# cboin1996/avddpg

Hardware: AMD Instinct MI355X
Metric: env-steps/sec + DDPG updates/sec, 4096x5-vehicle platoons (higher is better)
Workload: dtype f32-class (fp16 hi+lo operand pairs on the 16-bit matrix cores, f32 accumulate)

## Files before the change

### avddpg_amd/csrc/fsplit.hip

```cpp
#include <type_traits>

#include "fset_common.h"
#include "anchor.h"
#include "smooth.h"

namespace avd {
namespace fsplit {
using namespace fset;

struct ActorS {
    static constexpr int K = 256, KP = 256, NFT = 8, NKS = 16, LD = 264, NGT = 9, KG = 288;
    static constexpr bool critic = false;
};
struct CriticS {
    static constexpr int K = 304, KP = 320, NFT = 10, NKS = 19, LD = 312, NGT = 10, KG = 320;
    static constexpr bool critic = true;
};
constexpr int NGT_MAX = 10;

template <int I, int N, class F>
__device__ __forceinline__ void static_for(F&& f) {
    if constexpr (I < N) {
        f(std::integral_constant<int, I>{});
        static_for<I + 1, N>(f);
// ... 350 lines not shown
    b -= a.n_zero;
    const int which = b >= a.n_pack;
    pack_x_role<S>(a.pk, which, b - which * a.n_pack, a.pa.fflag + 4 * ((long)a.n_prep1 + b));
}

enum HeadMode { OUT_TANH = 0, OUT_TD = 1, HEAD_BOTH = 5, OUT_TANH_SAVE = 6 };
struct HeadArgs {
    unsigned long long* stamp;
    NetP net;
    int n_agents, n_sets;
    const f16x8* xf;
    const float* act;
    const float* act2;
    const float* r;
    const float* yin;
    const float* aw;
    float* out;
    unsigned* sm;
    float* g3;
    float* dmu;
    float* part_s;
    float* part_s2;
    float* part_m;
    float* tz;
    float gamma, high, inv_n;
    int* bad;
    int abl;
};
#ifndef HEAD_FAST
#define HEAD_FAST 5
#define HEAD_SLOW 3
#endif

template <int S, class NET, int MODE, bool HP = false, class... H>
__global__ __launch_bounds__(NT) void head_kernel(const HeadArgs p, H... hp) {
    constexpr int K = NET::K, NKS = NET::NKS, NFT = NET::NFT, LD = NET::LD;
    constexpr int NTH = NT;
    constexpr bool BOTH = (MODE == HEAD_BOTH);
    static_assert(!BOTH || NET::critic, "HEAD_BOTH is a critic mode");
    __shared__ __attribute__((aligned(16))) f16 wimg[2][H2 * LD];
    __shared__ __attribute__((aligned(16))) float b2s[H2];
    __shared__ __attribute__((aligned(16))) float c3s[H2];
    __shared__ __attribute__((aligned(16))) unsigned waps[BOTH ? 48 : 4];
    const int tid = threadIdx.x, w = tid >> 6, lane = tid & 63, r = lane & 31, h = lane >> 5, q = w >> 1, rh = w & 1;
    const int set = blockIdx.x % p.n_sets, j0 = blockIdx.x / p.n_sets, J = gridDim.x / p.n_sets, P = p.n_agents / p.n_sets;
#ifdef AVD_STAMP
    unsigned long long hacc[4] = {0, 0, 0, 0}, hlast = __builtin_amdgcn_s_memtime();
    const unsigned long long hstart = hlast;
#define HSTAMP(i) { const unsigned long long t_ = __builtin_amdgcn_s_memtime(); hacc[i] += t_ - hlast; hlast = t_; }
#else
#define HSTAMP(i)
#endif
    const float* vec = p.net.vec + (long)set * VEC;
    const f16x8* wf1 = p.net.wf1h + (long)set * NGT_MAX * 64 + lane;
    const f32x16 zero16 = {};
    const int ntile = j0 < P ? (P - j0 + J - 1) / J : 0;
    const int row = 32 * rh + r;
    f16x8 nx = {};
    float na = 0.f, nb = 0.f, ny = 0.f, nw = 1.f;
    auto fetch_in = [&](int k) {
        const int agent = (j0 + k * J) * p.n_sets + set;
        const long ri = (long)agent * TILE + row;
        nx = p.xf[2 * ri + h];
        if (NET::critic) na = p.act[ri];
        if (BOTH) nb = p.act2[ri];
        if (MODE == OUT_TD) ny = p.r[ri];
        if (BOTH) ny = p.yin[ri];
        if (BOTH && p.aw) nw = p.aw[agent];
    };
    constexpr int FAST = HEAD_FAST, SLOW = HEAD_SLOW, PERIOD = 2 * (FAST + SLOW);
    const int qs = __builtin_amdgcn_readfirstlane(q);
    const int cnt = qs < 2 ? FAST : SLOW, start = qs < 2 ? qs * FAST : 2 * FAST + (qs - 2) * SLOW;
    int k = start, pos = 0;
    auto next_tile = [&](int kk, int pp) { return pp + 1 == cnt ? kk + PERIOD - cnt + 1 : kk + 1; };
    const float SW = vec[2 * H2 + 1], d3 = vec[2 * H2];
    const float vb = vec[tid & (H2 - 1)], vc = vec[H2 + (tid & (H2 - 1))];
    unsigned wv = 0;
// ... 272 lines not shown
            if constexpr (HP) {
                if (h == 0) p.out[ri] = ty + hp_of(set, hp...).gamma * z;
            } else {
                if (h == 0) p.out[ri] = ty + p.gamma * z;
            }
        }
        HSTAMP(2);
#ifdef AVD_STAMP
        if (blockIdx.x == 16 && lane == 0 && p.stamp && (w == 0 || w == 4) && ui < 28)
            p.stamp[64 + (w >> 2) * 28 + ui] = hlast - hstart;
#endif
    }
#ifdef AVD_STAMP
    if (blockIdx.x == 16 && lane == 0 && p.stamp)
        for (int i = 0; i < 4; ++i) p.stamp[w * 8 + i] = hacc[i];
#endif
    if (watch >= 0x7f800000u) atomicOr(p.bad, 1);
    if (BOTH) {
#pragma unroll
        for (int o = 1; o < 32; o <<= 1) {
            Dacc += __shfl_xor(Dacc, o), Lacc += __shfl_xor(Lacc, o);
            Dacc2 += __shfl_xor(Dacc2, o), Lacc2 += __shfl_xor(Lacc2, o);
        }
#pragma unroll
        for (int o = 1; o < 64; o <<= 1) gmax = fmaxf(gmax, __shfl_xor(gmax, o));
        if (lane == 0) {
            const long slot = (long)blockIdx.x * 8 + w;
            p.part_m[slot] = gmax;
            p.part_s[slot * 2] = Dacc, p.part_s[slot * 2 + 1] = Lacc;
            p.part_s2[slot * 2] = Dacc2, p.part_s2[slot * 2 + 1] = Lacc2;
        }
    }
}

struct SeedArgs {
    int n_agents, n_sets;
    const float *dmu, *tz;
    float high;
    float *g3, *part_m, *part_s;
};
__global__ __launch_bounds__(NT) void actor_seed_kernel(const SeedArgs p) {
    const int tid = threadIdx.x, w = tid >> 6, lane = tid & 63;
    const int set = blockIdx.x % p.n_sets, j0 = blockIdx.x / p.n_sets, J = gridDim.x / p.n_sets, P = p.n_agents / p.n_sets;
    float gmax = 0.f, D = 0.f;
    for (int pi = j0 + w * J; pi < P; pi += 8 * J) {
        const long ri = (long)(pi * p.n_sets + set) * TILE + lane;
        const float t = p.tz[ri], g = p.dmu[ri] * p.high * (1.f - t * t);
        p.g3[ri] = g;
        gmax = fmaxf(gmax, fabsf(g));
        D += g;
    }
#pragma unroll
    for (int o = 1; o < 64; o <<= 1) gmax = fmaxf(gmax, __shfl_xor(gmax, o)), D += __shfl_xor(D, o);
    if (lane == 0) {
        p.part_m[(long)blockIdx.x * 8 + w] = gmax;
        p.part_s[((long)blockIdx.x * 8 + w) * 2] = D, p.part_s[((long)blockIdx.x * 8 + w) * 2 + 1] = 0.f;
    }
}

__device__ __forceinline__ float set_gscale(const float* part_m, int set, int n_sets, int J, float* red) {
    const int tid = threadIdx.x;
    float m = 0.f;
    for (int i = tid; i < J * 8; i += NT) m = fmaxf(m, part_m[((long)(i >> 3) * n_sets + set) * 8 + (i & 7)]);
#pragma unroll
    for (int o = 1; o < 64; o <<= 1) m = fmaxf(m, __shfl_xor(m, o));
    if ((tid & 63) == 0) red[tid >> 6] = m;
    __syncthreads();
    m = fmaxf(fmaxf(fmaxf(red[0], red[1]), fmaxf(red[2], red[3])), fmaxf(fmaxf(red[4], red[5]), fmaxf(red[6], red[7])));
    int e = 0;
    if (m > 0.f && !not_finite(m)) (void)frexpf(m, &e);
    const int k = e > 100 ? -100 : (e < -100 ? 100 : -e);
    return __uint_as_float(__builtin_amdgcn_readfirstlane(__float_as_uint(ldexpf(1.f, k))));
}

__device__ __forceinline__ unsigned mask_pair(unsigned d, int j, unsigned mj) { return __umul24(d & (0x10001u << j), mj); }
__device__ __forceinline__ void mask_chunk16(unsigned w, int c, unsigned m, uint4& lo, uint4& hi) {
    const unsigned d = w >> (8 * (c & 1));
    lo.x = mask_pair(d, 0, m), lo.y = mask_pair(d, 1, m >> 1), lo.z = mask_pair(d, 2, m >> 2), lo.w = mask_pair(d, 3, m >> 3);
    hi.x = mask_pair(d, 4, m >> 4), hi.y = mask_pair(d, 5, m >> 5), hi.z = mask_pair(d, 6, m >> 6), hi.w = mask_pair(d, 7, m >> 7);
}
__device__ __forceinline__ unsigned mask_one(float g3, bool signed_) { return signed_ && g3 < 0.f ? 0xbc00u : 0x3c00u; }

struct DwArgs {
    NetP net;
    int n_agents, n_sets;
    const float* x;
    const float* act;
    const float* g3;
    const float* part_m;
    const unsigned* sm;
    float* partG;
    int abl;
    unsigned long long* stamp;
};
template <int S, class NET>
__global__ __launch_bounds__(NT) void dw_kernel(const DwArgs p) {
    constexpr int KG = NET::KG, LDZ = 160;
    constexpr int XC = NET::critic ? 2 : 1;
    __shared__ __attribute__((aligned(16))) f16 smimg[2][TILE * LDZ];
    __shared__ __attribute__((aligned(16))) f16x8 fq[2][TILE * 2];
    __shared__ __attribute__((aligned(16))) f16x8 fa[2][TILE * 2];
    __shared__ float gred[8];
    const int tid = threadIdx.x, w = tid >> 6, lane = tid & 63, r = lane & 31, h = lane >> 5;
    const int set = blockIdx.x % p.n_sets, j0 = blockIdx.x / p.n_sets, J = gridDim.x / p.n_sets, P = p.n_agents / p.n_sets;
    float gsc;
    const f16x8* wf1 = p.net.wf1h + (long)set * NGT_MAX * 64 + lane;
    const int xt = NET::critic ? 8 + (w >> 2) : 8, xrh = NET::critic ? (w >> 1) & 1 : (w >> 2) & 1, xc0 = NET::critic ? 2 * (w & 1) : (w & 3);
    const f16x8 wf0 = wf1[64 * w], wfx = wf1[64 * xt];
    f32x16 G0[4], G1[XC];
    const f32x16 zero16 = {};
#pragma unroll
    for (int c = 0; c < 4; ++c) G0[c] = zero16;
#pragma unroll
    for (int c = 0; c < XC; ++c) G1[c] = zero16;

    const int srow = tid >> 3, sch = tid & 7, frow = tid >> 1, fh = tid & 1;
    unsigned ma = 0, mb = 0;
    float sx[4] = {0.f, 0.f, 0.f, 0.f}, sg = 0.f, sa = 0.f, ga = 0.f, gb = 0.f;
    auto fetch_m = [&](int pl, unsigned& m, float& g) {
        const long ri = (long)(((FSPLIT_ABL(p.abl) & 1) ? j0 : pl) * p.n_sets + set) * TILE + srow;
        m = p.sm[ri * 4 + (sch >> 1)];
        g = p.g3[ri];
    };
    auto fetch_x = [&](int pl) {
        if (pl >= P || tid >= 2 * TILE) return;
        const long ri = (long)(pl * p.n_sets + set) * TILE + frow;
        load_x<S>(p.x, ri, sx);
        sg = p.g3[ri];
        if (NET::critic) sa = p.act[ri];
    };
    auto stage_m = [&](int buf, unsigned m, float g) {
        uint4* dst = (uint4*)(smimg[buf] + srow * LDZ + 16 * sch);
        mask_chunk16(m, sch, mask_one(g, true), dst[0], dst[1]);
    };
    auto stage_x = [&](int pl, int buf) {
        if (pl >= P) return;
// ... 82 lines not shown
            __builtin_amdgcn_sched_barrier(0);
        }
        stage_m(buf ^ 1, m, g);
#pragma unroll
        for (int s = 0; s < 2; ++s) {
            const f16x8 hi = fragh(ah[4 * s], ah[4 * s + 1], ah[4 * s + 2], ah[4 * s + 3]);
            const f16x8 lo = fragh(al[4 * s], al[4 * s + 1], al[4 * s + 2], al[4 * s + 3]);
#pragma unroll
            for (int c = 0; c < XC; ++c) {
                f16x8 bx;
#pragma unroll
                for (int hf = 0; hf < 2; ++hf) {
                    const int R0 = 32 * xrh + 16 * s + 8 * hf + 4 * (g4 >> 1);
                    const f16x4 t = read_tr(smimg[buf] + (R0 + q) * LDZ + 32 * (xc0 + c) + 16 * (g4 & 1) + 4 * pp);
#pragma unroll
                    for (int j = 0; j < 4; ++j) bx[4 * hf + j] = t[j];
                }
                G1[c] = mfmah(hi, bx, G1[c]);
                G1[c] = mfmah(lo, bx, G1[c]);
            }
        }
        __builtin_amdgcn_sched_group_barrier(0x100, 4 * XC, 0);
#pragma unroll
        for (int i = 0; i < 4 * XC; ++i) {
            __builtin_amdgcn_sched_group_barrier(0x008, 1, 0);
            __builtin_amdgcn_sched_group_barrier(0x002, 6, 0);
        }
        __builtin_amdgcn_sched_group_barrier(0x200, 2, 0);
        __builtin_amdgcn_sched_barrier(0);
    };
    if (j0 < P) fetch_m(j0, ma, ga);
    fetch_x(j0);
    if (j0 + J < P) fetch_m(j0 + J, mb, gb);
    gsc = set_gscale(p.part_m, set, p.n_sets, J, gred);
    stage_m(0, ma, ga), stage_x(j0, 0);
    __syncthreads();
#ifdef AVD_STAMP
    unsigned long long tacc[4] = {0, 0, 0, 0}, tlast = __builtin_amdgcn_s_memtime();
#define STAMP(i) { const unsigned long long t_ = __builtin_amdgcn_s_memtime(); tacc[i] += t_ - tlast; tlast = t_; }
#else
#define STAMP(i)
#endif
    for (int pi = j0; pi < P; pi += 2 * J) {
        fetch_x(pi + J);
        if (pi + 2 * J < P) fetch_m(pi + 2 * J, ma, ga);
        STAMP(0);
        compute(0, mb, gb);
        STAMP(1);
        stage_x(pi + J, 1);
        STAMP(2);
        if (!(FSPLIT_ABL(p.abl) & 2)) __syncthreads();
        STAMP(3);
        if (pi + J < P) {
            fetch_x(pi + 2 * J);
            if (pi + 3 * J < P) fetch_m(pi + 3 * J, mb, gb);
            STAMP(0);
            compute(1, ma, ga);
            STAMP(1);
            stage_x(pi + 2 * J, 0);
            STAMP(2);
            if (!(FSPLIT_ABL(p.abl) & 2)) __syncthreads();
            STAMP(3);
        }
    }
#ifdef AVD_STAMP
    if (p.stamp && blockIdx.x == 16 && lane == 0)
        for (int i = 0; i < 4; ++i) p.stamp[w * 8 + i] = tacc[i];
#endif
    const float dsc = 1.f / (gsc * S1);
    float* comb = (float*)&smimg[0][0];
    const int cidx = NET::critic ? 2 * (w >> 2) + (w & 1) : (w & 3);
    if (xrh == 1) {
#pragma unroll
        for (int c = 0; c < XC; ++c)
#pragma unroll
            for (int k = 0; k < 16; ++k) comb[((cidx * XC + c) * 16 + k) * 64 + lane] = G1[c][k];
    }
    __syncthreads();
#pragma unroll
    for (int c = 0; c < 4; ++c) {
        float* dst = p.partG + ((long)blockIdx.x * KG + 32 * w) * H2 + 32 * c + r;
#pragma unroll
        for (int k = 0; k < 16; ++k) dst[(long)acc_row(k, h) * H2] = G0[c][k] * dsc;
    }
    if (xrh == 0) {
#pragma unroll
        for (int c = 0; c < XC; ++c) {
            float* dst = p.partG + ((long)blockIdx.x * KG + 32 * xt) * H2 + 32 * (xc0 + c) + r;
#pragma unroll
            for (int k = 0; k < 16; ++k) dst[(long)acc_row(k, h) * H2] = (G1[c][k] + comb[((cidx * XC + c) * 16 + k) * 64 + lane]) * dsc;
        }
    }
}

struct DxArgs {
    NetP net;
    int n_agents, n_sets;
    const f16x8* xfh;
    const float* act;
    int L_cWa, L_cba;
    const float* g3;
    const float* part_m;
    const unsigned* sm;
    float* partV;
    int abl;
    unsigned long long* stamp;
};
template <int S, class NET>
__global__ __launch_bounds__(NT) void dx_kernel(const DxArgs p) {
    constexpr int KP = NET::KP, LDZ = 136;
    constexpr float VSH = 1.f / 32.f;
    __shared__ __attribute__((aligned(16))) f16 smimg[2][TILE * LDZ];
    __shared__ __attribute__((aligned(16))) f16 xt[3][2][32 * 32];
    __shared__ __attribute__((aligned(16))) float g3s[3][TILE];
    __shared__ float gred[8];
    const int tid = threadIdx.x, w = __builtin_amdgcn_readfirstlane(tid >> 6), lane = tid & 63, r = lane & 31, h = lane >> 5, ft = w;
    const int set = blockIdx.x % p.n_sets, j0 = blockIdx.x / p.n_sets, J = gridDim.x / p.n_sets, P = p.n_agents / p.n_sets;
    const f32x16 zero16 = {};
    f16x8 wch[8], wcl[8];
    {
        const long at = ((long)set * KP + 32 * ft + r) * H2 + 8 * h;
#pragma unroll
        for (int s = 0; s < 8; ++s) wch[s] = *(const f16x8*)(p.net.Wchi + at + 16 * s), wcl[s] = *(const f16x8*)(p.net.Wclo + at + 16 * s);
    }
    const float swc = __uint_as_float(__builtin_amdgcn_readfirstlane(__float_as_uint(p.net.vec[(long)set * VEC + 2 * H2 + 2])));
    float gv, vs;
    const f16x8 wf = p.net.wf1h[((long)set * NGT_MAX + ft) * 64 + lane];
    f32x16 V = zero16;
    for (int i = tid; i < 3 * 2 * 32 * 32; i += NT) {
        const int k = (i >> 5) & 31;
        (&xt[0][0][0])[i] = (f16)(k == 8 ? 1.f : 0.f);
    }
    const int srow = tid >> 3, sch = tid & 7;
    unsigned dm = 0;
    float gn = 0.f, gs = 0.f;
    auto fetch = [&](int pl) {
        if (FSPLIT_ABL(p.abl) & 1) pl = j0;
        const long agent = (long)pl * p.n_sets + set;
        dm = p.sm[(agent * TILE + srow) * 4 + (sch >> 1)];
        if (NET::critic) gs = p.g3[agent * TILE + srow];
        if (tid < TILE) gn = p.g3[agent * TILE + tid];
    };
    auto stage = [&](int buf, int slot) {
        uint4* dst = (uint4*)(smimg[buf] + srow * LDZ + 16 * sch);
        mask_chunk16(dm, sch, mask_one(gs, NET::critic), dst[0], dst[1]);
        if (tid < TILE) g3s[slot][tid] = (NET::critic ? fabsf(gn) : gn) * gv;
    };
    f16x8 xfn0 = {}, xfn1 = {};
    auto fetch_x = [&](int pl) {
// ... 92 lines not shown
        if constexpr (has_prev) v_product(vh1, vl1, xb1);
        read_a(buf, 1, smf);
        read_img(xt[slot][0], xb0);
        dc1 = dc_product(smf);
        p11 = mfmah(xf1, wf, zero16);
        backward(slot, 0, dc0, p10, vh0, vl0);
        stage(buf ^ 1, nslot);
        stage_x(nslot);
        xf0 = xfn0, xf1 = xfn1;
        fetch(nn), fetch_x(nn);
        __builtin_amdgcn_sched_group_barrier(0x100, 16, 0);
#pragma unroll
        for (int i = 0; i < (has_prev ? 21 : 17); ++i) {
            __builtin_amdgcn_sched_group_barrier(0x008, 1, 0);
            __builtin_amdgcn_sched_group_barrier(0x002, 6, 0);
            __builtin_amdgcn_sched_group_barrier(0x200, 1, 0);
        }
        __builtin_amdgcn_sched_barrier(0);
        v_product(vh0, vl0, xb0);
        DXSTAMP(2);
        if (!(FSPLIT_ABL(p.abl) & 2)) __syncthreads();
        DXSTAMP(3);
    };
    unsigned dm0 = 0;
    float gn0 = 0.f, gs0 = 0.f;
    f16x8 xfa = {}, xfb = {};
    if (j0 < P) {
        fetch(j0), fetch_x(j0);
        dm0 = dm, gn0 = gn, gs0 = gs, xfa = xfn0, xfb = xfn1;
        const int n1 = j0 + J < P ? j0 + J : j0;
        fetch(n1), fetch_x(n1);
    }
    {
        const float gsc = set_gscale(p.part_m, set, p.n_sets, J, gred);
        gv = gsc * VSH, vs = gsc * swc * VSH;
    }
    if (j0 < P) {
        const unsigned dm1 = dm;
        const float gn1 = gn, gs1 = gs;
        const f16x8 xfc = xfn0, xfd = xfn1;
        dm = dm0, gn = gn0, gs = gs0, xfn0 = xfa, xfn1 = xfb;
        stage(0, 0), stage_x(0);
        xf0 = xfn0, xf1 = xfn1;
        dm = dm1, gn = gn1, gs = gs1, xfn0 = xfc, xfn1 = xfd;
    }
    __syncthreads();
    if (j0 < P) {
        iteration(std::false_type{}, j0, 0, 0);
        int buf = 1, slot = 1, pi = j0 + J;
        for (; pi < P; pi += J, buf ^= 1, slot = slot == 2 ? 0 : slot + 1) iteration(std::true_type{}, pi, buf, slot);
        const int pslot = slot == 0 ? 2 : slot - 1;
        f16x8 xb1[2];
        unsigned vh1[8], vl1[8];
        read_img(xt[pslot][1], xb1);
        backward(pslot, 1, dc1, p11, vh1, vl1);
        v_product(vh1, vl1, xb1);
    }
#ifdef AVD_STAMP
    if (p.stamp && blockIdx.x == 16 && lane == 0)
        for (int i = 0; i < 4; ++i) p.stamp[w * 8 + i] = dacc[i];
#endif
    const float ivs = 1.f / vs;
    if (r < 16) {
        float* pv = p.partV + ((long)blockIdx.x * KP + 32 * ft) * 16 + r;
#pragma unroll
        for (int k = 0; k < 16; ++k) pv[(long)acc_row(k, h) * 16] = V[k] * ivs;
    }
}

template <int S>
__global__ __launch_bounds__(NT) void dxa_kernel(const DxArgs p) {
    typedef CriticS NET;
    constexpr int KP = NET::KP;
    constexpr float VSH = 1.f / 32.f;
    __shared__ __attribute__((aligned(16))) float ga[8][2][2][32];
    __shared__ float comb[8][64][2];
    __shared__ float gred[8];
    const int tid = threadIdx.x, w = __builtin_amdgcn_readfirstlane(tid >> 6), lane = tid & 63, r = lane & 31, h = lane >> 5;
    const int rh = w & 1, ftl = (w >> 1) & 1, par = w >> 2;
    const int set = blockIdx.x % p.n_sets, j0 = blockIdx.x / p.n_sets, J = gridDim.x / p.n_sets, P = p.n_agents / p.n_sets;
    const f32x16 zero16 = {};
    const int ft = 8 + ftl, f = 32 * ftl + r;
    f16x8 wch[8], wcl[8];
    {
        const long at = ((long)set * KP + 32 * ft + r) * H2 + 8 * h;
#pragma unroll
        for (int s = 0; s < 8; ++s) wch[s] = *(const f16x8*)(p.net.Wchi + at + 16 * s), wcl[s] = *(const f16x8*)(p.net.Wclo + at + 16 * s);
    }
    const float swc = __uint_as_float(__builtin_amdgcn_readfirstlane(__float_as_uint(p.net.vec[(long)set * VEC + 2 * H2 + 2])));
    const float* th = p.net.th + (long)set * p.net.th_stride;
    const float wa = f < HA ? th[p.L_cWa + f] : 0.f, ba = f < HA ? th[p.L_cba + f] : 0.f;
    float Sa = 0.f, Sb = 0.f;
    const int ntile = j0 < P ? (P - j0 + J - 1) / J : 0;
    uint4 mA = {}, mB = {};
    float gA = 0.f, aA = 0.f, gB = 0.f, aB = 0.f;
#define DXA_FETCH(k_, m_, g_, a_)                                                                                   \
    {                                                                                                               \
        const long r0_ = (long)((j0 + (k_) * J) * p.n_sets + set) * TILE + 32 * rh;                                 \
        m_ = *(const uint4*)(p.sm + (r0_ + r) * 4);                                                                 \
        g_ = p.g3[r0_ + r], a_ = p.act[r0_ + r];                                                                    \
    }
#define DXA_PUT(buf_, g_, a_)                                                                                       \
    {                                                                                                               \
        if (h == 0) ga[w][buf_][0][r] = fabsf(g_) * gv, ga[w][buf_][1][r] = a_;                                     \
        __builtin_amdgcn_fence(__ATOMIC_RELEASE, "wavefront");                                                      \
        __builtin_amdgcn_wave_barrier();                                                                            \
    }
    auto unit = [&](int buf, const uint4 mw, float g) {
        f32x16 dc = zero16;
        const unsigned m = mask_one(g, true);
        const unsigned mwt[4] = {mw.x >> (4 * h), mw.y >> (4 * h), mw.z >> (4 * h), mw.w >> (4 * h)};
#pragma unroll
        for (int s = 0; s < 8; ++s) {
            const unsigned d = mwt[s >> 1] >> (8 * (s & 1));
            const f16x8 af = fragh(mask_pair(d, 0, m), mask_pair(d, 1, m >> 1), mask_pair(d, 2, m >> 2), mask_pair(d, 3, m >> 3));
            dc = mfmah(af, wch[s], dc), dc = mfmah(af, wcl[s], dc);
        }
        float sa = 0.f, sb = 0.f;
#pragma unroll
        for (int q = 0; q < 4; ++q) {
            const float4 gq = *(const float4*)(&ga[w][buf][0][8 * q + 4 * h]), aq = *(const float4*)(&ga[w][buf][1][8 * q + 4 * h]);
            const float gg[4] = {gq.x, gq.y, gq.z, gq.w}, av[4] = {aq.x, aq.y, aq.z, aq.w};
#pragma unroll
            for (int j = 0; j < 4; ++j) {
                const float m = fmaf(av[j], wa, ba) > 0.f ? dc[4 * q + j] * gg[j] : 0.f;
                sa = fmaf(m, av[j], sa);
                sb += m;
            }
        }
        Sa += sa, Sb += sb;
        __builtin_amdgcn_fence(__ATOMIC_ACQ_REL, "wavefront");
        __builtin_amdgcn_wave_barrier();
    };
    if (par < ntile) DXA_FETCH(par, mA, gA, aA);
    if (par + 2 < ntile) DXA_FETCH(par + 2, mB, gB, aB);
    const float gsc = set_gscale(p.part_m, set, p.n_sets, J, gred);
    const float gv = gsc * VSH, vs = gsc * swc * VSH;
    for (int k = par; k < ntile; k += 4) {
        DXA_PUT(0, gA, aA);
        {
            const uint4 mc = mA;
            const float gc = gA;
            if (k + 4 < ntile) DXA_FETCH(k + 4, mA, gA, aA);
            unit(0, mc, gc);
        }
        if (k + 2 < ntile) {
            DXA_PUT(1, gB, aB);
            const uint4 mc = mB;
            const float gc = gB;
            if (k + 6 < ntile) DXA_FETCH(k + 6, mB, gB, aB);
            unit(1, mc, gc);
        }
    }
#undef DXA_FETCH
#undef DXA_PUT
    comb[w][lane][0] = Sa, comb[w][lane][1] = Sb;
    __syncthreads();
    if (rh == 0 && par == 0 && h == 0) {
        const int ws[4] = {w, w + 1, w + 4, w + 5};
        float t[2] = {0.f, 0.f};
#pragma unroll
        for (int i = 0; i < 4; ++i)
#pragma unroll
            for (int c = 0; c < 2; ++c) t[c] += comb[ws[i]][r][c] + comb[ws[i]][32 + r][c];
        const float ivs = 1.f / vs;
        float* pv = p.partV + ((long)blockIdx.x * KP + 32 * ft + r) * 16;
#pragma unroll
        for (int c = 0; c < 9; ++c) pv[c] = c == 0 ? t[0] * ivs : (c == 8 ? t[1] * ivs : 0.f);
    }
}

struct Plan {
    int grid, J;
    size_t Whi[4], Wlo[4], Wchi[2], Wclo[2], wf1h[4], vec[4], wap, a2, y, mu, dmu, g3, sm, sma, tz, t1p, s2raw, xfs, xfs2, partHs[3], partM[2],
        partV[2], partG[2], bad, smax, fflag, total;
    int n_prep1, n_pack, n_fflag;
};
static Plan make_plan(int n_agents, int n_sets) {
    Plan pl;
    const int P = n_agents / n_sets;
    int J = cu_count() / n_sets;
    if (const char* e = AVD_DIAG_ENV("FSPLIT_J")) J = atoi(e);
    if (J < 1) J = 1;
    if (J > P) J = P;
    pl.J = J, pl.grid = J * n_sets;
    size_t o = 0;
    auto take = [&](size_t bytes) {
        const size_t at = o;
        o += (bytes + 255) / 256 * 256;
        return at;
    };
    for (int i = 0; i < 4; ++i) {
        const int K = (i & 1) ? CriticS::K : ActorS::K, KP = (i & 1) ? CriticS::KP : ActorS::KP;
        pl.Whi[i] = take(sizeof(f16) * (size_t)n_sets * H2 * K), pl.Wlo[i] = take(sizeof(f16) * (size_t)n_sets * H2 * K);
        pl.vec[i] = take(sizeof(float) * (size_t)n_sets * VEC);
        pl.wf1h[i] = take(16 * (size_t)n_sets * NGT_MAX * 64);
        if (i < 2) pl.Wchi[i] = take(sizeof(f16) * (size_t)n_sets * KP * H2), pl.Wclo[i] = take(sizeof(f16) * (size_t)n_sets * KP * H2);
    }
    pl.wap = take(4 * (size_t)n_sets * 48);
    const size_t rows = (size_t)n_agents * TILE;
    pl.a2 = take(4 * rows), pl.y = take(4 * rows), pl.mu = take(4 * rows), pl.dmu = take(4 * rows), pl.g3 = take(4 * rows);
    pl.sm = take(16 * rows);
    pl.sma = take(16 * rows);
    pl.tz = take(4 * rows);
    pl.t1p = take(2 * 4 * (size_t)n_sets * CriticS::K * H2), pl.s2raw = take(2 * 4 * (size_t)n_sets * H2);
    pl.xfs = take(32 * rows), pl.xfs2 = take(32 * rows);
    for (int i = 0; i < 2; ++i) {
        const int KP = i ? CriticS::KP : ActorS::KP, KG = i ? CriticS::KG : ActorS::KG;
        pl.partM[i] = take(4 * (size_t)pl.grid * 8);
        pl.partV[i] = take(4 * (size_t)pl.grid * KP * 16);
        pl.partG[i] = take(4 * (size_t)pl.grid * KG * H2);
    }
    for (int i = 0; i < 3; ++i) pl.partHs[i] = take(4 * (size_t)pl.grid * 8 * 2);
    pl.n_prep1 = (NGT_MAX * 4 * n_sets + 3) / 4, pl.n_pack = (int)((2 * rows + 255) / 256);
    pl.n_fflag = 4 * (pl.n_prep1 + 2 * pl.n_pack);
    pl.bad = take(sizeof(int));
    pl.smax = take(sizeof(unsigned) * 4 * (size_t)n_sets * SCALE_SLICES * 2);
    pl.fflag = take(sizeof(unsigned) * (size_t)pl.n_fflag);
    pl.total = o;
    return pl;
}
static int check_shape(const avd_mlp_layout* L, int n_agents, int n_sets, const char* who) {
    AVD_REQUIRE(L, "%s: null layout", who);
    if (L->H1 != H1 || L->H2 != H2 || L->Ha != HA || L->A != 1 || (L->S != 3 && L->S != 4) || L->B != TILE) {
        set_error("%s: serves the reference widths only (layer1 256, layer2 128, action layer 48, A = 1, S in {3, 4}, B = 64); "
                  "got H1=%d H2=%d Ha=%d A=%d S=%d B=%d (avd_learn_shared_bf16 takes other widths)",
                  who, L->H1, L->H2, L->Ha, L->A, L->S, L->B);
        return AVD_E_UNSUPPORTED;
    }
    AVD_REQUIRE(n_sets > 0 && n_sets <= 64 && n_agents > 0 && n_agents % n_sets == 0, "%s: n_agents=%d n_sets=%d", who, n_agents,
                n_sets);
    return AVD_OK;
}

// ... 11 lines not shown
        for (int w = 0; w < 8; ++w) {
            const unsigned long long* s = head_stamps() + 128 * ni + 8 * w;
            fprintf(stderr, "HSTAMP %-22s wave %d: start-up %8llu  unit-start %8llu  tiles %9llu  epilogue %8llu  start-up share %.4f\n", who[ni], w,
                    s[3], s[0], s[1], s[2], (double)s[3] / (double)(s[0] + s[1] + s[2] + s[3] + 1));
        }
}
#endif
template <int S, class... H>
static int run(int phases, const avd_mlp_layout& L, int n_agents, int n_sets, const float* theta, const float* stats, const float* theta_t,
               const float* stats_t, const float* s, const float* a, const float* r, const float* s2, const float* aw, float gamma,
               float high, float* grads, float* losses, unsigned char* ws, const Plan& pl, hipStream_t st, const AnchorArgs* an,
               const SmoothArgs* smo, H... hp) {
    PrepArgs pa;
    pa.L = L, pa.S = S, pa.theta = theta, pa.stats = stats, pa.theta_t = theta_t, pa.stats_t = stats_t;
    pa.wap = (unsigned*)(ws + pl.wap), pa.bad = (int*)(ws + pl.bad), pa.smax = (unsigned*)(ws + pl.smax);
    pa.fflag = (unsigned*)(ws + pl.fflag), pa.n_fflag = pl.n_fflag;
    NetP net[4];
    for (int i = 0; i < 4; ++i) {
        const bool critic = i & 1, target = i >= 2;
        pa.Whi[i] = (f16*)(ws + pl.Whi[i]), pa.Wlo[i] = (f16*)(ws + pl.Wlo[i]), pa.vec[i] = (float*)(ws + pl.vec[i]);
        pa.wf1h[i] = (f16x8*)(ws + pl.wf1h[i]);
        pa.Wchi[i] = i < 2 ? (f16*)(ws + pl.Wchi[i]) : nullptr, pa.Wclo[i] = i < 2 ? (f16*)(ws + pl.Wclo[i]) : nullptr;
        NetP& n = net[i];
        n.th = (target ? theta_t : theta) + (critic ? L.actor_size : 0), n.th_stride = L.theta_size;
        n.Whi = pa.Whi[i], n.Wlo = pa.Wlo[i], n.Wchi = pa.Wchi[i], n.Wclo = pa.Wclo[i], n.wf1h = pa.wf1h[i], n.vec = pa.vec[i];
        n.wap = pa.wap;
    }
    const int P = n_agents / n_sets;
    const float inv_n = 1.0f / ((float)P * TILE);
    const long nrows = (long)n_agents * TILE;
    f16x8 *xfs = (f16x8*)(ws + pl.xfs), *xfs2 = (f16x8*)(ws + pl.xfs2);
    int* bad = (int*)(ws + pl.bad);
    float *a2 = (float*)(ws + pl.a2), *y = (float*)(ws + pl.y), *mu = (float*)(ws + pl.mu), *dmu = (float*)(ws + pl.dmu);
    float* g3 = (float*)(ws + pl.g3);
    unsigned *sm = (unsigned*)(ws + pl.sm), *sma = (unsigned*)(ws + pl.sma);
    auto F = [&](size_t off) { return (float*)(ws + off); };
    const dim3 grid(pl.grid), block(NT);
    HeadArgs h;
    h.n_agents = n_agents, h.n_sets = n_sets, h.gamma = gamma, h.high = high, h.inv_n = inv_n, h.aw = aw, h.sm = sm, h.g3 = g3, h.dmu = dmu;
    h.act2 = nullptr, h.part_s2 = nullptr, h.stamp = nullptr, h.bad = bad, h.part_m = nullptr, h.tz = F(pl.tz), h.abl = 0;
    if (const char* e = AVD_DIAG_ENV("FSPLIT_ABL")) h.abl = atoi(e);
    auto head = [&](auto kern, int ni, const f16x8* x, const float* act, const float* rr, const float* yin, float* out, float* part_s,
                    auto... extra) {
        h.net = net[ni], h.xf = x, h.act = act, h.r = rr, h.yin = yin, h.out = out, h.part_s = part_s;
#ifdef AVD_STAMP
        h.stamp = head_stamps() + 128 * ni;
#endif
        hipLaunchKernelGGL(kern, grid, block, 0, st, h, extra...);
    };
    DwArgs dw;
    dw.n_agents = n_agents, dw.n_sets = n_sets, dw.sm = sm, dw.g3 = g3, dw.x = s, dw.stamp = nullptr, dw.abl = 0;
    if (const char* e = AVD_DIAG_ENV("FSPLIT_ABL")) dw.abl = atoi(e);
#ifdef AVD_STAMP
    static unsigned long long* d_stamp = nullptr;
    if (!d_stamp) (void)hipMalloc(&d_stamp, 128 * 8);
    dw.stamp = d_stamp;
#endif
    DxArgs dx;
    dx.n_agents = n_agents, dx.n_sets = n_sets, dx.sm = sm, dx.g3 = g3, dx.xfh = xfs, dx.stamp = nullptr, dx.L_cWa = dx.L_cba = 0;
    dx.abl = dw.abl;
#ifdef AVD_STAMP
    dx.stamp = d_stamp;
#endif
    FinArgs fa;
    fa.L = L, fa.n_sets = n_sets, fa.J = pl.J, fa.S = S, fa.nrh = 1, fa.theta = theta, fa.stats = stats, fa.grads = grads, fa.losses = losses;
    fa.inv_n = inv_n, fa.partLa = F(pl.partHs[2]), fa.bad = bad;
    for (int i = 0; i < 2; ++i)
        fa.partH[i] = nullptr, fa.partHs[i] = F(pl.partHs[i]), fa.partU[i] = nullptr, fa.partV[i] = F(pl.partV[i]),
        fa.partG[i] = F(pl.partG[i]), fa.c3[i] = F(pl.vec[i]);
    fa.t1_from_g[0] = fa.t1_from_g[1] = 1, fa.t1p = F(pl.t1p), fa.s2raw = F(pl.s2raw);
    if (phases & PH_CRITIC) {
        FrontArgs fr;
        fr.pa = pa, fr.grads = grads, fr.n_grads = (long)n_sets * L.theta_size, fr.n_sets = n_sets;
        fr.pk.x[0] = s, fr.pk.extra[0] = a, fr.pk.outh[0] = xfs, fr.pk.x[1] = s2, fr.pk.extra[1] = r, fr.pk.outh[1] = xfs2, fr.pk.rows = nrows;
        fr.n_scale = 4 * n_sets * SCALE_SLICES, fr.n_prep1 = pl.n_prep1, fr.n_pack = pl.n_pack;
        fr.n_zero = (int)((fr.n_grads + ZERO_PER_BLOCK - 1) / ZERO_PER_BLOCK);
        hipLaunchKernelGGL(front_kernel<S>, dim3((unsigned)(fr.n_scale + fr.n_prep1 + fr.n_zero + 2 * fr.n_pack)), dim3(256), 0, st, fr);
        hipLaunchKernelGGL(prep_kernel, dim3(H2, 4, n_sets), dim3(320), 0, st, pa);
        head(head_kernel<S, ActorS, OUT_TANH>, 2, xfs2, nullptr, nullptr, nullptr, a2, nullptr);
        if (smo) {
            SmoothArgs q = *smo;
            q.n_agents = n_agents, q.a2 = a2;
            launch_target_smooth(q, st);
        }
        if constexpr (sizeof...(H) > 0)
            head(head_kernel<S, CriticS, OUT_TD, true, H...>, 3, xfs2, a2, r, nullptr, y, nullptr, hp...);
        else
            head(head_kernel<S, CriticS, OUT_TD>, 3, xfs2, a2, r, nullptr, y, nullptr);
        h.sm = sma;
        head(head_kernel<S, ActorS, OUT_TANH_SAVE>, 0, xfs, nullptr, nullptr, nullptr, mu, nullptr);
        h.sm = sm;
        h.act2 = mu, h.part_s2 = F(pl.partHs[2]), h.part_m = F(pl.partM[1]);
        head(head_kernel<S, CriticS, HEAD_BOTH>, 1, xfs, a, nullptr, y, nullptr, F(pl.partHs[1]));
        dw.net = net[1], dw.act = a, dw.partG = F(pl.partG[1]), dw.part_m = F(pl.partM[1]);
        hipLaunchKernelGGL((dw_kernel<S, CriticS>), grid, block, 0, st, dw);
        dx.net = net[1], dx.partV = F(pl.partV[1]), dx.act = a, dx.part_m = F(pl.partM[1]);
        hipLaunchKernelGGL((dx_kernel<S, CriticS>), grid, block, 0, st, dx);
        dx.L_cWa = L.cWa, dx.L_cba = L.cba;
        hipLaunchKernelGGL((dxa_kernel<S>), grid, block, 0, st, dx);
        if (phases == PH_CRITIC) launch_finalize(fa, st, 1, 1);
    }
    if (phases & PH_ACTOR) {
        SeedArgs sd;
        sd.n_agents = n_agents, sd.n_sets = n_sets, sd.dmu = dmu, sd.tz = F(pl.tz), sd.high = high, sd.g3 = g3, sd.part_m = F(pl.partM[0]),
        sd.part_s = F(pl.partHs[0]);
        if (an) {
            AnchorArgs q = *an;
            q.n_agents = n_agents, q.n_sets = n_sets, q.S = S, q.J = pl.J, q.dmu = dmu, q.tz = sd.tz, q.high = high, q.g3 = g3;
            q.part_m = sd.part_m, q.part_s = sd.part_s, q.mu = mu, q.s = s, q.aw = aw, q.inv_n = inv_n, q.c = 2.f * an->weight * inv_n;
            q.bad = bad;
            launch_anchor_seed(q, pl.grid, st);
        } else
            hipLaunchKernelGGL(actor_seed_kernel, grid, block, 0, st, sd);
        dw.sm = sma, dx.sm = sma;
        dw.net = net[0], dw.act = nullptr, dw.partG = F(pl.partG[0]), dw.part_m = F(pl.partM[0]);
        hipLaunchKernelGGL((dw_kernel<S, ActorS>), grid, block, 0, st, dw);
        dx.net = net[0], dx.partV = F(pl.partV[0]), dx.act = nullptr, dx.part_m = F(pl.partM[0]), dx.L_cWa = dx.L_cba = 0;
        hipLaunchKernelGGL((dx_kernel<S, ActorS>), grid, block, 0, st, dx);
        if (phases == PH_ACTOR) launch_finalize(fa, st, 0, 1);
        else launch_finalize(fa, st, 0, 2);
    }
#ifdef AVD_STAMP
    if (AVD_DIAG_ENV("FSPLIT_STAMPS")) print_head_stamps(st);
#endif
    return check_launch("avd_learn_set_split");
}

}
}

using namespace avd;

namespace avd { namespace fsplit {
constexpr long MFMA_PER_TILE = 2 * (200 + 238 + 200 + 314)
                               + 8 * (2 + 32 + 1 + 2 * 2 * 2)
                               + 8 * (2 + 32 + 1 + 2 * 1 * 2)
                               + 2 * 8 * (32 + 2 + 8)
                               + 4 * 16;
static_assert(MFMA_PER_TILE == 3296, "update DESIGN.md 3.4 and the count above together");
}}
extern "C" int avd_learn_set_split_mfma_count(const avd_mlp_layout* lay, int n_agents, int n_sets, unsigned long long* mfma_32x32x16) {
    int rc = fsplit::check_shape(lay, n_agents, n_sets, "avd_learn_set_split_mfma_count");
    if (rc) return rc;
    AVD_REQUIRE(mfma_32x32x16, "avd_learn_set_split_mfma_count: null pointer");
    *mfma_32x32x16 = (unsigned long long)fsplit::MFMA_PER_TILE * (unsigned long long)n_agents;
    return AVD_OK;
}
// ... 122 lines not shown
```

Baseline: 2.195 million.

## Fuse forward head passes and backward dw/dx passes into two persistent kernels

Each head, seed, dw, dx and dxa kernel becomes a device body that takes a shared-memory pointer. Two new kernels, forward_kernel and backward_kernel, run those bodies one after another inside a single launch, with block barriers between phases and the shared memory sized for the largest phase. The actor seed now runs in the forward pass, before the critic backward pass, so it writes its gradient to a separate g3a buffer to avoid overwriting data the critic still needs. This removes about eight launches and their tail gaps per update step. In exchange, the shared-memory footprint and register pressure of the fused kernels may reduce occupancy. The fused path is used only when both phases run without anchor, smoothing or extra hooks.

After: 2.261 million (median of 6 runs). +3.0%, better.

```diff
diff --git a/avddpg_amd/csrc/fsplit.hip b/avddpg_amd/csrc/fsplit.hip
--- a/avddpg_amd/csrc/fsplit.hip
+++ b/avddpg_amd/csrc/fsplit.hip
@@ -406,17 +406,21 @@
 #define HEAD_SLOW 3
 #endif
 
+template <class NET, int MODE>
+constexpr int head_lds_bytes() {
+    return 2 * H2 * NET::LD * (int)sizeof(f16) + 2 * H2 * (int)sizeof(float) + (MODE == HEAD_BOTH ? 48 : 4) * (int)sizeof(unsigned);
+}
 template <int S, class NET, int MODE, bool HP = false, class... H>
-__global__ __launch_bounds__(NT) void head_kernel(const HeadArgs p, H... hp) {
+__device__ __forceinline__ void head_body(const HeadArgs& p, unsigned char* lds, const int tid, H... hp) {
     constexpr int K = NET::K, NKS = NET::NKS, NFT = NET::NFT, LD = NET::LD;
     constexpr int NTH = NT;
     constexpr bool BOTH = (MODE == HEAD_BOTH);
     static_assert(!BOTH || NET::critic, "HEAD_BOTH is a critic mode");
-    __shared__ __attribute__((aligned(16))) f16 wimg[2][H2 * LD];
-    __shared__ __attribute__((aligned(16))) float b2s[H2];
-    __shared__ __attribute__((aligned(16))) float c3s[H2];
-    __shared__ __attribute__((aligned(16))) unsigned waps[BOTH ? 48 : 4];
-    const int tid = threadIdx.x, w = tid >> 6, lane = tid & 63, r = lane & 31, h = lane >> 5, q = w >> 1, rh = w & 1;
+    f16(*wimg)[H2 * LD] = (f16(*)[H2 * LD]) lds;
+    float* b2s = (float*)(lds + 2 * H2 * LD * sizeof(f16));
+    float* c3s = b2s + H2;
+    unsigned* waps = (unsigned*)(c3s + H2);
+    const int w = tid >> 6, lane = tid & 63, r = lane & 31, h = lane >> 5, q = w >> 1, rh = w & 1;
     const int set = blockIdx.x % p.n_sets, j0 = blockIdx.x / p.n_sets, J = gridDim.x / p.n_sets, P = p.n_agents / p.n_sets;
 #ifdef AVD_STAMP
     unsigned long long hacc[4] = {0, 0, 0, 0}, hlast = __builtin_amdgcn_s_memtime();
@@ -755,6 +759,11 @@
         }
     }
 }
+template <int S, class NET, int MODE, bool HP = false, class... H>
+__global__ __launch_bounds__(NT) void head_kernel(const HeadArgs p, H... hp) {
+    __shared__ __attribute__((aligned(16))) unsigned char lds[head_lds_bytes<NET, MODE>()];
+    head_body<S, NET, MODE, HP, H...>(p, lds, threadIdx.x, hp...);
+}
 
 struct SeedArgs {
     int n_agents, n_sets;
@@ -762,8 +771,8 @@
     float high;
     float *g3, *part_m, *part_s;
 };
-__global__ __launch_bounds__(NT) void actor_seed_kernel(const SeedArgs p) {
-    const int tid = threadIdx.x, w = tid >> 6, lane = tid & 63;
+__device__ __forceinline__ void seed_body(const SeedArgs& p, const int tid) {
+    const int w = tid >> 6, lane = tid & 63;
     const int set = blockIdx.x % p.n_sets, j0 = blockIdx.x / p.n_sets, J = gridDim.x / p.n_sets, P = p.n_agents / p.n_sets;
     float gmax = 0.f, D = 0.f;
     for (int pi = j0 + w * J; pi < P; pi += 8 * J) {
@@ -780,9 +789,9 @@
         p.part_s[((long)blockIdx.x * 8 + w) * 2] = D, p.part_s[((long)blockIdx.x * 8 + w) * 2 + 1] = 0.f;
     }
 }
-
-__device__ __forceinline__ float set_gscale(const float* part_m, int set, int n_sets, int J, float* red) {
-    const int tid = threadIdx.x;
+__global__ __launch_bounds__(NT) void actor_seed_kernel(const SeedArgs p) { seed_body(p, threadIdx.x); }
+
+__device__ __forceinline__ float set_gscale(const float* part_m, int set, int n_sets, int J, float* red, const int tid) {
     float m = 0.f;
     for (int i = tid; i < J * 8; i += NT) m = fmaxf(m, part_m[((long)(i >> 3) * n_sets + set) * 8 + (i & 7)]);
 #pragma unroll
@@ -816,15 +825,17 @@
     int abl;
     unsigned long long* stamp;
 };
+constexpr int DW_LDZ = 160;
+constexpr int DW_LDS_BYTES = 2 * TILE * DW_LDZ * (int)sizeof(f16) + 2 * 2 * TILE * 2 * 16 + 8 * (int)sizeof(float);
 template <int S, class NET>
-__global__ __launch_bounds__(NT) void dw_kernel(const DwArgs p) {
-    constexpr int KG = NET::KG, LDZ = 160;
+__device__ __forceinline__ void dw_body(const DwArgs& p, unsigned char* lds, const int tid) {
+    constexpr int KG = NET::KG, LDZ = DW_LDZ;
     constexpr int XC = NET::critic ? 2 : 1;
-    __shared__ __attribute__((aligned(16))) f16 smimg[2][TILE * LDZ];
-    __shared__ __attribute__((aligned(16))) f16x8 fq[2][TILE * 2];
-    __shared__ __attribute__((aligned(16))) f16x8 fa[2][TILE * 2];
-    __shared__ float gred[8];
-    const int tid = threadIdx.x, w = tid >> 6, lane = tid & 63, r = lane & 31, h = lane >> 5;
+    f16(*smimg)[TILE * LDZ] = (f16(*)[TILE * LDZ]) lds;
+    f16x8(*fq)[TILE * 2] = (f16x8(*)[TILE * 2])(lds + 2 * TILE * LDZ * sizeof(f16));
+    f16x8(*fa)[TILE * 2] = fq + 2;
+    float* gred = (float*)(fa + 2);
+    const int w = tid >> 6, lane = tid & 63, r = lane & 31, h = lane >> 5;
     const int set = blockIdx.x % p.n_sets, j0 = blockIdx.x / p.n_sets, J = gridDim.x / p.n_sets, P = p.n_agents / p.n_sets;
     float gsc;
     const f16x8* wf1 = p.net.wf1h + (long)set * NGT_MAX * 64 + lane;
@@ -973,7 +984,7 @@
     if (j0 < P) fetch_m(j0, ma, ga);
     fetch_x(j0);
     if (j0 + J < P) fetch_m(j0 + J, mb, gb);
-    gsc = set_gscale(p.part_m, set, p.n_sets, J, gred);
+    gsc = set_gscale(p.part_m, set, p.n_sets, J, gred, tid);
     stage_m(0, ma, ga), stage_x(j0, 0);
     __syncthreads();
 #ifdef AVD_STAMP
@@ -1033,6 +1044,11 @@
         }
     }
 }
+template <int S, class NET>
+__global__ __launch_bounds__(NT) void dw_kernel(const DwArgs p) {
+    __shared__ __attribute__((aligned(16))) unsigned char lds[DW_LDS_BYTES];
+    dw_body<S, NET>(p, lds, threadIdx.x);
+}
 
 struct DxArgs {
     NetP net;
@@ -1047,15 +1063,17 @@
     int abl;
     unsigned long long* stamp;
 };
+constexpr int DX_LDZ = 136;
+constexpr int DX_LDS_BYTES = 2 * TILE * DX_LDZ * (int)sizeof(f16) + 3 * 2 * 32 * 32 * (int)sizeof(f16) + 3 * TILE * (int)sizeof(float) + 8 * (int)sizeof(float);
 template <int S, class NET>
-__global__ __launch_bounds__(NT) void dx_kernel(const DxArgs p) {
-    constexpr int KP = NET::KP, LDZ = 136;
+__device__ __forceinline__ void dx_body(const DxArgs& p, unsigned char* lds, const int tid) {
+    constexpr int KP = NET::KP, LDZ = DX_LDZ;
     constexpr float VSH = 1.f / 32.f;
-    __shared__ __attribute__((aligned(16))) f16 smimg[2][TILE * LDZ];
-    __shared__ __attribute__((aligned(16))) f16 xt[3][2][32 * 32];
-    __shared__ __attribute__((aligned(16))) float g3s[3][TILE];
-    __shared__ float gred[8];
-    const int tid = threadIdx.x, w = __builtin_amdgcn_readfirstlane(tid >> 6), lane = tid & 63, r = lane & 31, h = lane >> 5, ft = w;
+    f16(*smimg)[TILE * LDZ] = (f16(*)[TILE * LDZ]) lds;
+    f16(*xt)[2][32 * 32] = (f16(*)[2][32 * 32])(lds + 2 * TILE * LDZ * sizeof(f16));
+    float(*g3s)[TILE] = (float(*)[TILE])(xt + 3);
+    float* gred = (float*)(g3s + 3);
+    const int w = __builtin_amdgcn_readfirstlane(tid >> 6), lane = tid & 63, r = lane & 31, h = lane >> 5, ft = w;
     const int set = blockIdx.x % p.n_sets, j0 = blockIdx.x / p.n_sets, J = gridDim.x / p.n_sets, P = p.n_agents / p.n_sets;
     const f32x16 zero16 = {};
     f16x8 wch[8], wcl[8];
@@ -1214,7 +1232,7 @@
         fetch(n1), fetch_x(n1);
     }
     {
-        const float gsc = set_gscale(p.part_m, set, p.n_sets, J, gred);
+        const float gsc = set_gscale(p.part_m, set, p.n_sets, J, gred, tid);
         gv = gsc * VSH, vs = gsc * swc * VSH;
     }
     if (j0 < P) {
@@ -1249,16 +1267,22 @@
         for (int k = 0; k < 16; ++k) pv[(long)acc_row(k, h) * 16] = V[k] * ivs;
     }
 }
-
+template <int S, class NET>
+__global__ __launch_bounds__(NT) void dx_kernel(const DxArgs p) {
+    __shared__ __attribute__((aligned(16))) unsigned char lds[DX_LDS_BYTES];
+    dx_body<S, NET>(p, lds, threadIdx.x);
+}
+
+constexpr int DXA_LDS_BYTES = (8 * 2 * 2 * 32 + 8 * 64 * 2 + 8) * (int)sizeof(float);
 template <int S>
-__global__ __launch_bounds__(NT) void dxa_kernel(const DxArgs p) {
+__device__ __forceinline__ void dxa_body(const DxArgs& p, unsigned char* lds, const int tid) {
     typedef CriticS NET;
     constexpr int KP = NET::KP;
     constexpr float VSH = 1.f / 32.f;
-    __shared__ __attribute__((aligned(16))) float ga[8][2][2][32];
-    __shared__ float comb[8][64][2];
-    __shared__ float gred[8];
-    const int tid = threadIdx.x, w = __builtin_amdgcn_readfirstlane(tid >> 6), lane = tid & 63, r = lane & 31, h = lane >> 5;
+    float(*ga)[2][2][32] = (float(*)[2][2][32]) lds;
+    float(*comb)[64][2] = (float(*)[64][2])(ga + 8);
+    float* gred = (float*)(comb + 8);
+    const int w = __builtin_amdgcn_readfirstlane(tid >> 6), lane = tid & 63, r = lane & 31, h = lane >> 5;
     const int rh = w & 1, ftl = (w >> 1) & 1, par = w >> 2;
     const int set = blockIdx.x % p.n_sets, j0 = blockIdx.x / p.n_sets, J = gridDim.x / p.n_sets, P = p.n_agents / p.n_sets;
     const f32x16 zero16 = {};
@@ -1316,7 +1340,7 @@
     };
     if (par < ntile) DXA_FETCH(par, mA, gA, aA);
     if (par + 2 < ntile) DXA_FETCH(par + 2, mB, gB, aB);
-    const float gsc = set_gscale(p.part_m, set, p.n_sets, J, gred);
+    const float gsc = set_gscale(p.part_m, set, p.n_sets, J, gred, tid);
     const float gv = gsc * VSH, vs = gsc * swc * VSH;
     for (int k = par; k < ntile; k += 4) {
         DXA_PUT(0, gA, aA);
@@ -1351,10 +1375,67 @@
         for (int c = 0; c < 9; ++c) pv[c] = c == 0 ? t[0] * ivs : (c == 8 ? t[1] * ivs : 0.f);
     }
 }
+template <int S>
+__global__ __launch_bounds__(NT) void dxa_kernel(const DxArgs p) {
+    __shared__ __attribute__((aligned(16))) unsigned char lds[DXA_LDS_BYTES];
+    dxa_body<S>(p, lds, threadIdx.x);
+}
+
+__device__ __forceinline__ void phase_seam() {
+    __builtin_amdgcn_sched_barrier(0);
+    __syncthreads();
+    __builtin_amdgcn_sched_barrier(0);
+}
+__device__ __forceinline__ int phase_tid() {
+    int t = threadIdx.x;
+    asm volatile("" : "+v"(t));
+    __builtin_assume(t >= 0 && t < NT);
+    return t;
+}
+struct FwdArgs {
+    HeadArgs tanh_t, td, tanh_save, both;
+    SeedArgs seed;
+};
+struct BwdArgs {
+    DwArgs dw_c;
+    DxArgs dx_c, dxa;
+    DwArgs dw_a;
+    DxArgs dx_a;
+};
+constexpr int FWD_LDS_BYTES = head_lds_bytes<CriticS, HEAD_BOTH>();
+static_assert(FWD_LDS_BYTES >= head_lds_bytes<ActorS, OUT_TANH_SAVE>() && FWD_LDS_BYTES >= head_lds_bytes<CriticS, OUT_TD>(), "the largest phase");
+constexpr int BWD_LDS_BYTES = DW_LDS_BYTES > DX_LDS_BYTES ? DW_LDS_BYTES : DX_LDS_BYTES;
+static_assert(BWD_LDS_BYTES >= DXA_LDS_BYTES, "the largest phase");
+template <int S>
+__global__ __launch_bounds__(NT) void forward_kernel(const FwdArgs a) {
+    __shared__ __attribute__((aligned(16))) unsigned char lds[FWD_LDS_BYTES];
+    head_body<S, ActorS, OUT_TANH>(a.tanh_t, lds, phase_tid());
+    phase_seam();
+    head_body<S, CriticS, OUT_TD>(a.td, lds, phase_tid());
+    phase_seam();
+    head_body<S, ActorS, OUT_TANH_SAVE>(a.tanh_save, lds, phase_tid());
+    phase_seam();
+    head_body<S, CriticS, HEAD_BOTH>(a.both, lds, phase_tid());
+    phase_seam();
+    seed_body(a.seed, phase_tid());
+}
+template <int S>
+__global__ __launch_bounds__(NT) void backward_kernel(const BwdArgs a) {
+    __shared__ __attribute__((aligned(16))) unsigned char lds[BWD_LDS_BYTES];
+    dw_body<S, CriticS>(a.dw_c, lds, phase_tid());
+    phase_seam();
+    dx_body<S, CriticS>(a.dx_c, lds, phase_tid());
+    phase_seam();
+    dxa_body<S>(a.dxa, lds, phase_tid());
+    phase_seam();
+    dw_body<S, ActorS>(a.dw_a, lds, phase_tid());
+    phase_seam();
+    dx_body<S, ActorS>(a.dx_a, lds, phase_tid());
+}
 
 struct Plan {
     int grid, J;
-    size_t Whi[4], Wlo[4], Wchi[2], Wclo[2], wf1h[4], vec[4], wap, a2, y, mu, dmu, g3, sm, sma, tz, t1p, s2raw, xfs, xfs2, partHs[3], partM[2],
+    size_t Whi[4], Wlo[4], Wchi[2], Wclo[2], wf1h[4], vec[4], wap, a2, y, mu, dmu, g3, g3a, sm, sma, tz, t1p, s2raw, xfs, xfs2, partHs[3], partM[2],
         partV[2], partG[2], bad, smax, fflag, total;
     int n_prep1, n_pack, n_fflag;
 };
@@ -1382,6 +1463,7 @@
     pl.wap = take(4 * (size_t)n_sets * 48);
     const size_t rows = (size_t)n_agents * TILE;
     pl.a2 = take(4 * rows), pl.y = take(4 * rows), pl.mu = take(4 * rows), pl.dmu = take(4 * rows), pl.g3 = take(4 * rows);
+    pl.g3a = take(4 * rows);
     pl.sm = take(16 * rows);
     pl.sma = take(16 * rows);
     pl.tz = take(4 * rows);
@@ -1459,7 +1541,7 @@
     f16x8 *xfs = (f16x8*)(ws + pl.xfs), *xfs2 = (f16x8*)(ws + pl.xfs2);
     int* bad = (int*)(ws + pl.bad);
     float *a2 = (float*)(ws + pl.a2), *y = (float*)(ws + pl.y), *mu = (float*)(ws + pl.mu), *dmu = (float*)(ws + pl.dmu);
-    float* g3 = (float*)(ws + pl.g3);
+    float *g3 = (float*)(ws + pl.g3), *g3a = (float*)(ws + pl.g3a);
     unsigned *sm = (unsigned*)(ws + pl.sm), *sma = (unsigned*)(ws + pl.sma);
     auto F = [&](size_t off) { return (float*)(ws + off); };
     const dim3 grid(pl.grid), block(NT);
@@ -1467,13 +1549,16 @@
     h.n_agents = n_agents, h.n_sets = n_sets, h.gamma = gamma, h.high = high, h.inv_n = inv_n, h.aw = aw, h.sm = sm, h.g3 = g3, h.dmu = dmu;
     h.act2 = nullptr, h.part_s2 = nullptr, h.stamp = nullptr, h.bad = bad, h.part_m = nullptr, h.tz = F(pl.tz), h.abl = 0;
     if (const char* e = AVD_DIAG_ENV("FSPLIT_ABL")) h.abl = atoi(e);
-    auto head = [&](auto kern, int ni, const f16x8* x, const float* act, const float* rr, const float* yin, float* out, float* part_s,
-                    auto... extra) {
+    auto head_args = [&](int ni, const f16x8* x, const float* act, const float* rr, const float* yin, float* out, float* part_s) {
         h.net = net[ni], h.xf = x, h.act = act, h.r = rr, h.yin = yin, h.out = out, h.part_s = part_s;
 #ifdef AVD_STAMP
         h.stamp = head_stamps() + 128 * ni;
 #endif
-        hipLaunchKernelGGL(kern, grid, block, 0, st, h, extra...);
+        return h;
+    };
+    auto head = [&](auto kern, int ni, const f16x8* x, const float* act, const float* rr, const float* yin, float* out, float* part_s,
+                    auto... extra) {
+        hipLaunchKernelGGL(kern, grid, block, 0, st, head_args(ni, x, act, rr, yin, out, part_s), extra...);
     };
     DwArgs dw;
     dw.n_agents = n_agents, dw.n_sets = n_sets, dw.sm = sm, dw.g3 = g3, dw.x = s, dw.stamp = nullptr, dw.abl = 0;
@@ -1496,6 +1581,14 @@
         fa.partH[i] = nullptr, fa.partHs[i] = F(pl.partHs[i]), fa.partU[i] = nullptr, fa.partV[i] = F(pl.partV[i]),
         fa.partG[i] = F(pl.partG[i]), fa.c3[i] = F(pl.vec[i]);
     fa.t1_from_g[0] = fa.t1_from_g[1] = 1, fa.t1p = F(pl.t1p), fa.s2raw = F(pl.s2raw);
+    bool fused = phases == PH_BOTH && !an && !smo && sizeof...(H) == 0;
+#ifdef AVD_STAMP
+    fused = false;
+#endif
+    if (AVD_DIAG_ENV("FSPLIT_UNFUSED")) fused = false;
+    SeedArgs sd;
+    sd.n_agents = n_agents, sd.n_sets = n_sets, sd.dmu = dmu, sd.tz = F(pl.tz), sd.high = high, sd.g3 = g3a, sd.part_m = F(pl.partM[0]),
+    sd.part_s = F(pl.partHs[0]);
     if (phases & PH_CRITIC) {
         FrontArgs fr;
         fr.pa = pa, fr.grads = grads, fr.n_grads = (long)n_sets * L.theta_size, fr.n_sets = n_sets;
@@ -1504,6 +1597,34 @@
         fr.n_zero = (int)((fr.n_grads + ZERO_PER_BLOCK - 1) / ZERO_PER_BLOCK);
         hipLaunchKernelGGL(front_kernel<S>, dim3((unsigned)(fr.n_scale + fr.n_prep1 + fr.n_zero + 2 * fr.n_pack)), dim3(256), 0, st, fr);
         hipLaunchKernelGGL(prep_kernel, dim3(H2, 4, n_sets), dim3(320), 0, st, pa);
+    }
+    if (fused) {
+        FwdArgs fw;
+        fw.tanh_t = head_args(2, xfs2, nullptr, nullptr, nullptr, a2, nullptr);
+        fw.td = head_args(3, xfs2, a2, r, nullptr, y, nullptr);
+        h.sm = sma;
+        fw.tanh_save = head_args(0, xfs, nullptr, nullptr, nullptr, mu, nullptr);
+        h.sm = sm;
+        h.act2 = mu, h.part_s2 = F(pl.partHs[2]), h.part_m = F(pl.partM[1]);
+        fw.both = head_args(1, xfs, a, nullptr, y, nullptr, F(pl.partHs[1]));
+        fw.seed = sd;
+        hipLaunchKernelGGL(forward_kernel<S>, grid, block, 0, st, fw);
+        BwdArgs bw;
+        dw.net = net[1], dw.act = a, dw.partG = F(pl.partG[1]), dw.part_m = F(pl.partM[1]);
+        bw.dw_c = dw;
+        dx.net = net[1], dx.partV = F(pl.partV[1]), dx.act = a, dx.part_m = F(pl.partM[1]);
+        bw.dx_c = dx;
+        dx.L_cWa = L.cWa, dx.L_cba = L.cba;
+        bw.dxa = dx;
+        dw.sm = sma, dw.g3 = g3a, dw.net = net[0], dw.act = nullptr, dw.partG = F(pl.partG[0]), dw.part_m = F(pl.partM[0]);
+        bw.dw_a = dw;
+        dx.sm = sma, dx.g3 = g3a, dx.net = net[0], dx.partV = F(pl.partV[0]), dx.act = nullptr, dx.part_m = F(pl.partM[0]), dx.L_cWa = dx.L_cba = 0;
+        bw.dx_a = dx;
+        hipLaunchKernelGGL(backward_kernel<S>, grid, block, 0, st, bw);
+        launch_finalize(fa, st, 0, 2);
+        return check_launch("avd_learn_set_split");
+    }
+    if (phases & PH_CRITIC) {
         head(head_kernel<S, ActorS, OUT_TANH>, 2, xfs2, nullptr, nullptr, nullptr, a2, nullptr);
         if (smo) {
             SmoothArgs q = *smo;
@@ -1528,18 +1649,15 @@
         if (phases == PH_CRITIC) launch_finalize(fa, st, 1, 1);
     }
     if (phases & PH_ACTOR) {
-        SeedArgs sd;
-        sd.n_agents = n_agents, sd.n_sets = n_sets, sd.dmu = dmu, sd.tz = F(pl.tz), sd.high = high, sd.g3 = g3, sd.part_m = F(pl.partM[0]),
-        sd.part_s = F(pl.partHs[0]);
         if (an) {
             AnchorArgs q = *an;
-            q.n_agents = n_agents, q.n_sets = n_sets, q.S = S, q.J = pl.J, q.dmu = dmu, q.tz = sd.tz, q.high = high, q.g3 = g3;
+            q.n_agents = n_agents, q.n_sets = n_sets, q.S = S, q.J = pl.J, q.dmu = dmu, q.tz = sd.tz, q.high = high, q.g3 = g3a;
             q.part_m = sd.part_m, q.part_s = sd.part_s, q.mu = mu, q.s = s, q.aw = aw, q.inv_n = inv_n, q.c = 2.f * an->weight * inv_n;
             q.bad = bad;
             launch_anchor_seed(q, pl.grid, st);
         } else
             hipLaunchKernelGGL(actor_seed_kernel, grid, block, 0, st, sd);
-        dw.sm = sma, dx.sm = sma;
+        dw.sm = sma, dx.sm = sma, dw.g3 = g3a, dx.g3 = g3a;
         dw.net = net[0], dw.act = nullptr, dw.partG = F(pl.partG[0]), dw.part_m = F(pl.partM[0]);
         hipLaunchKernelGGL((dw_kernel<S, ActorS>), grid, block, 0, st, dw);
         dx.net = net[0], dx.partV = F(pl.partV[0]), dx.act = nullptr, dx.part_m = F(pl.partM[0]), dx.L_cWa = dx.L_cba = 0;
```
